# oppo-us-research/PoP-Net

Measured on AMD Instinct MI355X. Metric: depth-frames/sec end-to-end (480x640), higher is better.
Workload: dtype bf16

## Files before the change

### include/popnet_hip.h

```cpp
#ifndef POPNET_HIP_H
#define POPNET_HIP_H

#include <stddef.h>
#include <stdint.h>

#ifdef __cplusplus
extern "C" {
#endif

#define PN_ABI_VERSION 1

enum pn_status {
    PN_OK = 0,
    PN_ERR_INVALID = -1,
    PN_ERR_HIP = -2,
    PN_ERR_STATE = -3,
    PN_ERR_UNSUPPORTED = -4
};

enum pn_precision {
    PN_PREC_F32 = 0,
    PN_PREC_BF16 = 1,
    PN_PREC_BF16X3 = 2
};
// ... 16 lines not shown
int pn_abi_version(void);
int pn_build_experiments(void);
int pn_mfma_sustained(pn_ctx *ctx, double seconds, int waves_per_simd, double *tflops, double *in_kernel_ghz, void *hip_stream);
pn_ctx *pn_create(int device_id);
void pn_destroy(pn_ctx *ctx);
int pn_last_error(pn_ctx *ctx, char *buf, size_t buf_len);

int pn_preprocess(pn_ctx *ctx, const void *depth_dev, int depth_dtype, int B, int H, int W,
                  float *out_dev, int S, float depth_max, float depth_mean, float depth_std,
                  void *hip_stream);

pn_net *pn_net_create(pn_ctx *ctx, int kind, int num_parts, int a, int input_dim);
void pn_net_destroy(pn_net *net);
int pn_net_set_tensor(pn_net *net, const char *name, const float *host_data,
                      const int64_t *shape, int ndim);
int pn_net_finalize(pn_net *net, int precision, int max_batch, int in_h, int in_w);

int pn_rtpose_forward(pn_net *net, const float *x_dev, int B, float *paf_dev, float *heat_dev,
                      float *z_dev, void *hip_stream);
int pn_yolo_forward(pn_net *net, const float *x_dev, int B, float *out_dev, void *hip_stream);
int pn_rtpose_forward_frames(pn_net *net, const void *depth_dev, int depth_dtype, int B, int H, int W, float depth_max,
                             float depth_mean, float depth_std, float *paf_dev, float *heat_dev, float *z_dev,
                             void *hip_stream);
int pn_yolo_forward_frames(pn_net *net, const void *depth_dev, int depth_dtype, int B, int H, int W, float depth_max,
                           float depth_mean, float depth_std, float *out_dev, void *hip_stream);
int pn_net_read_activation(pn_net *net, const char *name, int B, float *host_out,
                           size_t host_elems, void *hip_stream);
int pn_net_copy_activation(pn_net *net, const char *name, int B, float *dev_out, void *hip_stream);
int pn_net_forward_partial(pn_net *net, const float *x_dev, int B, int nsteps, void *hip_stream);
int pn_net_forward_frames_partial(pn_net *net, const void *depth_dev, int depth_dtype, int B, int H, int W, float depth_max,
                                  float depth_mean, float depth_std, int nsteps, void *hip_stream);
int pn_net_num_steps(pn_net *net);
int pn_net_step_info(pn_net *net, int k, char *out, size_t cap);
int pn_conv_level_plan_info(pn_ctx *ctx, int precision, int max_batch, int num_cus, int B, int H, int W, int together, int nconv,
                            const int *cout, const int *cin, const int *ks, const int *stride, char *out, size_t cap);
int pn_conv_has_instance(int prec, int ks, int stride, int pitch, int cfg);
double pn_net_flops_per_frame(pn_net *net);
int pn_net_lock(pn_net *net, int locked);
int pn_net_profile_begin(pn_net *net);
int pn_net_profile_end(pn_net *net, double *conv_ms, int64_t *conv_launches, double *conv_flops,
                       double *other_ms, int64_t *other_launches);
int pn_net_profile_kernel(pn_net *net, int rank, char *name, size_t name_cap, double *ms,
                          int64_t *launches, double *flops);

#define PN_NUM_JOINTS 15
#define PN_NUM_LIMBS 14
#define PN_MAX_PEAKS_PER_JOINT 32
#define PN_MAX_PEAKS (PN_NUM_JOINTS * PN_MAX_PEAKS_PER_JOINT)
#define PN_MAX_CONN_PER_LIMB PN_MAX_PEAKS_PER_JOINT
#define PN_MAX_PERSONS 32

#define PN_FRAME_OVERFLOW_PEAKS 1u
#define PN_FRAME_OVERFLOW_PERSONS 2u

#define PN_Z_READOUT_HEAT_WEIGHTED 0
#define PN_Z_READOUT_CELL 1

typedef struct pn_parse_cfg {
    float thresh_heatmap;
    float thresh_paf;
    int   num_intermed_pts;
    int   downsample;
    int   input_size;
    int   w_org, h_org;
    double fx, fy, cx, cy;
    float depth_mean, depth_std;
// ... 276 lines not shown
```

### popnet_amd/_lib.py

```python
import ctypes as C
import os

import numpy as np

_HERE = os.path.dirname(os.path.abspath(__file__))
LIB_PATH = os.environ.get("POPNET_LIB_PATH") or os.path.join(_HERE, "libpopnet_hip.so")

PN_OK = 0
PN_PREC_F32, PN_PREC_BF16, PN_PREC_BF16X3 = 0, 1, 2
PN_NET_RTPOSE_LIGHT3D, PN_NET_YOLO_POSENET, PN_NET_A2J = 0, 1, 2
PN_DEPTH_F16, PN_DEPTH_F32, PN_DEPTH_NET = 0, 1, 2

PN_NUM_JOINTS = 15
PN_NUM_LIMBS = 14
PN_MAX_PEAKS_PER_JOINT = 32
PN_MAX_PEAKS = PN_NUM_JOINTS * PN_MAX_PEAKS_PER_JOINT
PN_MAX_PERSONS = 32
PN_YOLO_MAX_DET = 64
PN_PLAN_FORWARD, PN_PLAN_DGRAD, PN_PLAN_DGRAD_STRIDED, PN_PLAN_WGRAD = 0, 1, 2, 3
PN_FRAME_OVERFLOW_PEAKS, PN_FRAME_OVERFLOW_PERSONS = 1, 2


class PopnetError(RuntimeError):
    pass
# ... 65 lines not shown

PN_WIRE_MAX_PERSONS = 16
POSE_WIRE_DTYPE = np.dtype([
    ("n_persons", np.int32), ("status", np.uint32),
    ("person_joint", np.int16, (PN_WIRE_MAX_PERSONS, PN_NUM_JOINTS)),
    ("vals", np.float32, (PN_WIRE_MAX_PERSONS, PN_NUM_JOINTS, 6)),
], align=True)

_lib = None

_vp, _i, _f, _d, _sz = C.c_void_p, C.c_int, C.c_float, C.c_double, C.c_size_t
_SIGNATURES = {
    "pn_abi_version": (_i, []),
    "pn_build_experiments": (_i, []),
    "pn_mfma_sustained": (_i, [_vp, _d, _i, C.POINTER(_d), C.POINTER(_d), _vp]),
    "pn_create": (_vp, [_i]),
    "pn_destroy": (None, [_vp]),
    "pn_last_error": (_i, [_vp, C.c_char_p, _sz]),
    "pn_preprocess": (_i, [_vp, _vp, _i, _i, _i, _i, _vp, _i, _f, _f, _f, _vp]),
    "pn_net_create": (_vp, [_vp, _i, _i, _i, _i]),
    "pn_net_destroy": (None, [_vp]),
    "pn_net_set_tensor": (_i, [_vp, C.c_char_p, _vp, C.POINTER(C.c_int64), _i]),
    "pn_net_finalize": (_i, [_vp, _i, _i, _i, _i]),
    "pn_rtpose_forward": (_i, [_vp, _vp, _i, _vp, _vp, _vp, _vp]),
    "pn_yolo_forward": (_i, [_vp, _vp, _i, _vp, _vp]),
    "pn_rtpose_forward_frames": (_i, [_vp, _vp, _i, _i, _i, _i, _f, _f, _f, _vp, _vp, _vp, _vp]),
    "pn_yolo_forward_frames": (_i, [_vp, _vp, _i, _i, _i, _i, _f, _f, _f, _vp, _vp]),
    "pn_net_read_activation": (_i, [_vp, C.c_char_p, _i, _vp, _sz, _vp]),
    "pn_net_copy_activation": (_i, [_vp, C.c_char_p, _i, _vp, _vp]),
    "pn_net_forward_partial": (_i, [_vp, _vp, _i, _i, _vp]),
    "pn_net_forward_frames_partial": (_i, [_vp, _vp, _i, _i, _i, _i, _f, _f, _f, _i, _vp]),
    "pn_net_num_steps": (_i, [_vp]),
    "pn_net_step_info": (_i, [_vp, _i, C.c_char_p, _sz]),
    "pn_conv_level_plan_info": (_i, [_vp] + [_i] * 8 + [_vp] * 4 + [C.c_char_p, _sz]),
    "pn_conv_has_instance": (_i, [_i] * 5),
    "pn_net_flops_per_frame": (_d, [_vp]),
    "pn_net_lock": (_i, [_vp, _i]),
    "pn_parse_reserve": (_i, [_vp, _i]),
    "pn_net_profile_begin": (_i, [_vp]),
    "pn_net_profile_end": (_i, [_vp, C.POINTER(_d), C.POINTER(C.c_int64), C.POINTER(_d), C.POINTER(_d), C.POINTER(C.c_int64)]),
    "pn_net_profile_kernel": (_i, [_vp, _i, C.c_char_p, _sz, C.POINTER(C.c_double), C.POINTER(C.c_int64), C.POINTER(C.c_double)]),
    "pn_parse_cfg_default": (None, [C.POINTER(ParseCfg)]),
    "pn_parse_paf": (_i, [_vp, _vp, _vp, _vp, _i, _i, _i, C.POINTER(ParseCfg), _vp, _vp]),
    "pn_parse_paf_wire": (_i, [_vp, _vp, _vp, _vp, _i, _i, _i, C.POINTER(ParseCfg), _vp, _vp, _vp]),
    "pn_target_cfg_default": (None, [C.POINTER(TargetCfg)]),
    "pn_compose_depth": (_i, [_vp, _vp, _vp, _vp, _vp, _i, _i, _i, _i, _i, _f, _vp, _vp]),
    "pn_compose_bg": (_i, [_vp, _vp, _vp, _vp, _i, _i, _i, _i, _vp, _vp]),
    "pn_rasterize_targets": (_i, [_vp, _vp, _vp, _vp, _i, _i, _vp, C.POINTER(TargetCfg), _vp, _vp, _vp, _vp, _vp]),
    "pn_sizeof_augment_item": (_sz, []),
    "pn_sizeof_parse_cfg": (_sz, []),
    "pn_augment_resize": (_i, [_vp, _vp, _vp, _vp, _i, _i, _i, _vp, _i, _f, _f, _f, _vp]),
    "pn_train_set_precision": (_i, [_vp, _i]),
    "pn_train_ws_keep": (_i, [_vp, _i]),
    "pn_train_pack_cache": (_i, [_vp, _i]),
    "pn_train_pack_refresh": (_i, [_vp, _vp]),
    "pn_conv2d_forward": (_i, [_vp, _vp, _vp, _vp, _vp] + [_i] * 9 + [_vp]),
    "pn_conv2d_dgrad": (_i, [_vp, _vp, _vp, _vp] + [_i] * 8 + [_vp]),
    "pn_conv2d_wgrad": (_i, [_vp, _vp, _vp, _vp, _vp] + [_i] * 8 + [_vp]),
    "pn_bn_train_forward": (_i, [_vp] * 10 + [_f, _f] + [_i] * 4 + [_vp]),
    "pn_bn_train_backward": (_i, [_vp] * 8 + [_i] * 4 + [_vp] * 4 + [_i, _vp]),
    "pn_avgpool3s2_forward": (_i, [_vp, _vp, _vp, _i, _i, _i, _vp]),
    "pn_avgpool3s2_backward": (_i, [_vp, _vp, _vp, _i, _i, _i, _vp]),
    "pn_head_forward": (_i, [_vp, _vp, _vp, _vp] + [_i] * 4 + [_vp, _vp, _i, _vp, _vp]),
    "pn_head_backward": (_i, [_vp, _vp, _vp, _vp, _vp] + [_i] * 5 + [_vp, _vp]),
    "pn_slice_copy": (_i, [_vp, _vp, _i, _vp] + [_i] * 5 + [_vp]),
    "pn_sgd_nesterov": (_i, [_vp, _vp, _vp, _vp, C.c_size_t, _f, _f, _f, _i, _f, _vp]),
# ... 154 lines not shown
```

### popnet_amd/csrc/api.hip

```cpp
#pragma clang fp contract(off)
#include <cmath>
#include <cstdarg>
#include <cstdio>
#include <cstdlib>
#include <cstring>
#include "pn_internal.h"
#include "preproc_pixel.h"

template <typename TIN>
__global__ void preprocess_kernel(const TIN *__restrict__ depth, float *__restrict__ out, int B, int H, int W, int S,
                                  double scale_x, double scale_y, float dmax, float mean, float stdv) {
    const unsigned pix = blockIdx.x * blockDim.x + threadIdx.x;
    if (pix >= (unsigned)(S * S)) return;
    const int b = blockIdx.y;
    const int dy = (int)(pix / (unsigned)S);
    const int dx = (int)(pix - (unsigned)dy * (unsigned)S);
    const size_t gid = (size_t)b * S * S + pix;

    out[gid] = pn_preproc_pixel(depth + (size_t)b * H * W, H, W, dy, dx, scale_x, scale_y, dmax, mean, stdv);
}

PnSwitches pn_read_switches() {
    auto set = [](const char *name) { return getenv(name) != nullptr; };
    auto num = [](const char *name, int unset) { const char *e = getenv(name); return e ? atoi(e) : unset; };
    auto is = [](const char *name, const char *value) { const char *e = getenv(name); return e && !strcmp(e, value); };
    PnSwitches s;
    s.no_conv3 = set("POPNET_NO_CONV3");
    s.conv3_rpg8 = set("POPNET_CONV3_RPG8");
    s.conv3_pt14 = num("POPNET_CONV3_PT14", 0);
    s.conv3_nbuf2 = set("POPNET_CONV3_NBUF2");
    s.generic_c64_off = num("POPNET_GENERIC_C64", 1) == 0;
    if (set("POPNET_CONV4")) s.conv4 = num("POPNET_CONV4", 0) == 0 ? 0 : 1;
    s.no_mix = set("POPNET_NO_MIX");
    s.no_bblock = set("POPNET_NO_BBLOCK");
    s.bblock_x3 = num("POPNET_BBLOCK_X3", 0) != 0;
    s.bb64_static = set("POPNET_BB64_STATIC");
    s.bb64_halves = num("POPNET_BB64_HALVES", 1) == 2 ? 2 : 1;
    if (set("POPNET_BB64_STRIP")) { const int v = num("POPNET_BB64_STRIP", 0); s.bb64_strip = v == 1 || v == 2 ? v : 0; }
    s.no_tailfuse = set("POPNET_NO_TAILFUSE");
    s.no_poolfuse = set("POPNET_NO_POOLFUSE");
    s.no_stempool = set("POPNET_NO_STEMPOOL");
    s.no_embed3 = set("POPNET_NO_EMBED3");
    s.train_x3_wide = set("POPNET_TRAIN_X3_WIDE");
    s.train_wgrad_novec = set("POPNET_TRAIN_WGRAD_NOVEC");
    s.trainx_one_stream = num("POPNET_TRAINX_STREAMS", 0) == 1;
    s.trainx_stem_handover = set("POPNET_TRAINX_STEM_HANDOVER");
    s.trainx_stem_gather = is("POPNET_TRAINX_STEM_FWD", "gather");
    s.trainx_stem_bn_separate = is("POPNET_TRAINX_STEM_BN", "separate");
    s.trainx_stem_depth = num("POPNET_TRAINX_STEM_DEPTH", 2);
    s.trainx_pack_gather = is("POPNET_TRAINX_PACK", "gather");
    s.trainx_legacy_wgrad = is("POPNET_TRAINX_WGRAD", "legacy");
    return s;
}

extern "C" {

int pn_abi_version(void) { return PN_ABI_VERSION; }
int pn_build_experiments(void) { return 0; }

pn_ctx *pn_create(int device_id) {
    pn_ctx *ctx = new pn_ctx();
    ctx->device = device_id;
    int ndev = 0;
    hipError_t e = hipGetDeviceCount(&ndev);
    if (e != hipSuccess || device_id < 0 || device_id >= ndev) {
        char buf[256];
        snprintf(buf, sizeof buf, "pn_create: device %d not available (%d devices, %s)", device_id, ndev,
                 hipGetErrorString(e));
        ctx->err = buf;
        ctx->device = -1;
        return ctx;
    }
    hipDeviceProp_t prop;
    if (hipGetDeviceProperties(&prop, device_id) == hipSuccess) ctx->num_cus = prop.multiProcessorCount;
    return ctx;
// ... 85 lines not shown
```

### popnet_amd/csrc/conv_mfma.hip

```cpp
#include "pn_internal.h"
#include "conv_inst_table.h"

int pn_cfg_couts(int cfg) {
    switch (cfg) {
        case PN_CFG_C128: return 128;
        case PN_CFG_C64: return 64;
        case PN_CFG_C64W: return 64;
        case PN_CFG_C32: return 32;
        default: return 16;
    }
}


int pn_cfg_pixels(int cfg) { return cfg == PN_CFG_C128 ? 112 : (cfg == PN_CFG_C64W ? 224 : 128); }

size_t pn_conv_lds_bytes(int prec, int ks, int stride, int pitch, int R, int dil) {
    size_t pixb = prec == PN_PREC_BF16 ? 128 : 256;
    size_t rows = (size_t)(R - 1) * stride + (size_t)(ks - 1) * dil + 1;
    return rows * pitch * pixb;
}

extern "C" int pn_conv_has_instance(int prec, int ks, int stride, int pitch, int cfg) {
    if (prec != PN_PREC_BF16 && prec != PN_PREC_F32) return 0;
#define PN_HAS_CASE(KS, ST, PITCH, CFG) \
    if (ks == KS && stride == ST && pitch == PITCH && cfg == CFG) return 1;
    PN_CONV_INSTANCES(PN_HAS_CASE)
#undef PN_HAS_CASE
    return 0;
}

int pn_conv_has_instance_d2(int prec, int ks, int stride, int pitch, int cfg) {
    if (prec != PN_PREC_BF16 && prec != PN_PREC_F32) return 0;
#define PN_HAS_CASE(KS, ST, PITCH, CFG) \
    if (ks == KS && stride == ST && pitch == PITCH && cfg == CFG) return 1;
    PN_CONV_INSTANCES_D2(PN_HAS_CASE)
#undef PN_HAS_CASE
    return 0;
}

int pn_launch_conv_part0(pn_ctx *ctx, const ConvLaunch &L, hipStream_t stream);
int pn_launch_conv_d2_part0(pn_ctx *ctx, const ConvLaunch &L, hipStream_t stream);
int pn_launch_conv_d2_part1(pn_ctx *ctx, const ConvLaunch &L, hipStream_t stream);
int pn_launch_conv_acc_part0(pn_ctx *ctx, const ConvLaunch &L, hipStream_t stream);
int pn_launch_conv_acc_part1(pn_ctx *ctx, const ConvLaunch &L, hipStream_t stream);
int pn_launch_conv_acc_part2(pn_ctx *ctx, const ConvLaunch &L, hipStream_t stream);
int pn_launch_conv_part1(pn_ctx *ctx, const ConvLaunch &L, hipStream_t stream);
int pn_launch_conv_part2(pn_ctx *ctx, const ConvLaunch &L, hipStream_t stream);
int pn_launch_conv_part3(pn_ctx *ctx, const ConvLaunch &L, hipStream_t stream);

int pn_launch_conv(pn_ctx *ctx, const ConvLaunch &L, hipStream_t stream) {
    int rc;
    if (L.kern == 4) return pn_launch_conv4(ctx, L, stream);
    if (L.kern == 3) return pn_launch_conv3(ctx, L, stream);
    if (L.acc) {
        if (L.prec == PN_PREC_F32 && (L.dil == 1 || L.dil == 2)) {
            if ((rc = pn_launch_conv_acc_part0(ctx, L, stream)) != 1) return rc;
            if ((rc = pn_launch_conv_acc_part1(ctx, L, stream)) != 1) return rc;
            if ((rc = pn_launch_conv_acc_part2(ctx, L, stream)) != 1) return rc;
        }
        return pn_set_error(ctx, PN_ERR_UNSUPPORTED, "no blocked-accumulation conv kernel for prec=%d ks=%d stride=%d dilation=%d pitch=%d cfg=%d", L.prec, L.ks, L.stride, L.dil, L.pitch, L.cfg);
    }
    if (L.dil != 1) {
        if (L.dil == 2 && (rc = pn_launch_conv_d2_part0(ctx, L, stream)) != 1) return rc;
        if (L.dil == 2 && (rc = pn_launch_conv_d2_part1(ctx, L, stream)) != 1) return rc;
        return pn_set_error(ctx, PN_ERR_UNSUPPORTED, "no conv kernel for prec=%d ks=%d stride=%d dilation=%d pitch=%d cfg=%d", L.prec, L.ks, L.stride, L.dil, L.pitch, L.cfg);
    }
    if ((rc = pn_launch_conv_part0(ctx, L, stream)) != 1) return rc;
    if ((rc = pn_launch_conv_part1(ctx, L, stream)) != 1) return rc;
    if ((rc = pn_launch_conv_part2(ctx, L, stream)) != 1) return rc;
    if ((rc = pn_launch_conv_part3(ctx, L, stream)) != 1) return rc;
    return pn_set_error(ctx, PN_ERR_UNSUPPORTED, "no conv kernel for prec=%d ks=%d stride=%d pitch=%d cfg=%d", L.prec, L.ks,
                        L.stride, L.pitch, L.cfg);
}

int pn_conv_stage_maxpx(int prec, int ks, int stride, int pitch, int cfg) {
    if (cfg == PN_CFG_C64W) return 0;
    const int maxpx = stride != 1 ? 0 : (ks == 1 ? 128 : (pitch <= 32 ? 192 : (pitch <= 64 ? 288 : 360)));
    const int nch = prec == PN_PREC_BF16 ? 8 : 16;
    const int raw = (maxpx * nch + 255) / 256;
    return raw <= 12 ? maxpx : 0;
}
```

### popnet_amd/csrc/net_api.hip

```cpp
#include <cstdarg>
#include <cstdio>
#include <cstring>
#include "net_internal.h"

using namespace pnnet;

namespace {
std::string geom_json(int prec, bool x3, const ConvGeom &g, int H, int W, int cout, int cin_chunks, int B) {
    ConvProblem P;
    memset(&P, 0, sizeof P);
    pn_fill_conv_problem(P, {nullptr, H, W, 0, 64, 0}, B, cin_chunks, cout, g, prec, x3);
    char t[384];
    snprintf(t, sizeof t, "\"kernel\": \"%s\", \"kern\": %d, \"cfg\": %d, \"pitch\": %d, \"R\": %d, \"Wt\": %d, \"wc\": %d, \"wp\": %d, \"nbuf\": %d, \"pt\": %d, \"rpg\": %d, "
             "\"tiles_x\": %d, \"tiles_per_img\": %d, \"cout_blocks\": %d, \"nblocks\": %d, \"lds_two\": %d",
             (g.dil != 1 ? pn_conv_kernel_label_dil(prec, g.ks, g.stride, g.pitch, g.cfg, g.dil) : pn_conv_kernel_label(prec, g.kern, false, g.ks, g.stride, g.pitch, g.cfg, g.wc, g.wp, g.nbuf, g.pt, g.rpg)).c_str(), g.kern, g.cfg, g.pitch, g.R, g.Wt, g.wc,
             g.wp, g.nbuf, g.pt, g.rpg, P.tiles_x, P.tiles_per_img, P.cout_blocks, P.nblocks, P.lds_two);
    return t;
}

int forward_entry(pn_net *n, int kind, bool pointers_ok, bool state = true) {
    if (!n) return PN_ERR_INVALID;
    pn_ctx *ctx = n->ctx;
    if (n->kind != kind)
        return pn_set_error(ctx, PN_ERR_INVALID, "not %s net", kind == PN_NET_RTPOSE_LIGHT3D ? "an rtpose_light3d" : kind == PN_NET_YOLO_POSENET ? "a YoloPoseNet" : "an A2J");
// ... 238 lines not shown
        else js += "null";
        const Buf &ib = n->bufs[c.in_buf];
        js += ", " + geom_json(n->prec, n->x3, c, ib.H, ib.W, c.cout, c.cin_chunks, n->last_B > 0 ? n->last_B : n->max_batch);
        if (c.dil != 1) add(", \"dil\": %d", c.dil);
        if (c.acc) add(", \"blocked_acc\": %d", c.acc);
        js += "}";
    };
    if (k == -1) {
        add("{\"prec\": \"%s\", \"in_h\": %d, \"in_w\": %d, \"input_dim\": %d, \"max_batch\": %d, \"steps\": %zu, \"bufs\": [",
            n->x3 ? "bf16x3" : n->prec == PN_PREC_BF16 ? "bf16" : "fp32", n->in_h, n->in_w, n->input_dim, n->max_batch, n->steps.size());
        for (size_t i = 0; i < n->bufs.size(); ++i) add(i ? ", [%d, %d, %d]" : "[%d, %d, %d]", n->bufs[i].H, n->bufs[i].W, n->bufs[i].plane);
        js += "]}";
    } else {
        const Step &st = n->steps[k];
        static const char *types[] = {"stem", "pool", "conv", "bblock"};
        add("{\"type\": \"%s\", \"kernel\": \"%s\"", types[(int)st.type], step_label(n, st).c_str());
        if (st.type == Step::STEM) add(", \"cin\": %d, \"out_buf\": %d, \"pool_buf\": %d", st.stem_cin, st.out_buf, st.stem_pool_buf);
        else if (st.type == Step::POOL) add(", \"mode\": %d, \"in_buf\": %d, \"out_buf\": %d, \"C\": %d, \"out_coff\": %d", st.pool.mode, st.pool.in_buf, st.pool.out_buf, st.pool.C, st.pool.out_coff);
        else {
            js += ", \"convs\": [";
            for (size_t i = 0; i < st.conv_ids.size(); ++i) {
                if (i) js += ", ";
                conv(st.conv_ids[i]);
            }
            js += "]";
        }
        js += "}";
    }
    if (js.size() + 1 > cap) return pn_set_error(ctx, PN_ERR_INVALID, "pn_net_step_info: %zu bytes needed", js.size() + 1);
    memcpy(out, js.c_str(), js.size() + 1);
    return PN_OK;
}

int pn_conv_level_plan_info(pn_ctx *ctx, int precision, int max_batch, int num_cus, int B, int H, int W, int together, int nconv, const int *cout,
                            const int *cin, const int *ks, const int *stride, char *out, size_t cap) {
    if (!ctx) return PN_ERR_INVALID;
    if (!out || !cout || !cin || !ks || !stride || nconv < 1 || nconv > 3 || max_batch < 1 || B < 1 || B > max_batch || num_cus < 1 || H < 1 || W < 1 ||
        (precision != PN_PREC_F32 && precision != PN_PREC_BF16 && precision != PN_PREC_BF16X3))
        return pn_set_error(ctx, PN_ERR_INVALID, "pn_conv_level_plan_info: bad arguments");
    for (int i = 0; i < nconv; ++i)
        if (cout[i] < 1 || cin[i] < 1 || (ks[i] != 1 && ks[i] != 3) || (stride[i] != 1 && stride[i] != 2))
            return pn_set_error(ctx, PN_ERR_INVALID, "pn_conv_level_plan_info: convolution %d: bad arguments", i);
    const bool x3 = precision == PN_PREC_BF16X3;
    const int prec = x3 ? PN_PREC_BF16 : precision;
    const PnSwitches sw = pn_read_switches();
    std::vector<PnLevelConv> lv(nconv);
    for (int i = 0; i < nconv; ++i) {
        lv[i].H = H; lv[i].W = W; lv[i].rows = cout[i]; lv[i].ks = ks[i]; lv[i].stride = stride[i];
        lv[i].cin_gt64 = cin[i] > 64;
    }
    if (together) pn_plan_level(lv, max_batch, x3, sw.conv4);
    std::string js = "{\"convs\": [";
    for (int i = 0; i < nconv; ++i) {
        const int cin_chunks = ((x3 ? 3 : 1) * cin[i] + 63) / 64;
        ConvGeom g;
        g.ks = ks[i]; g.stride = stride[i];
        pn_plan_conv_kernel(prec, max_batch, num_cus, H, W, cout[i], cin_chunks, lv[i].wc_min, lv[i].nbuf_min, lv[i].k4_level, sw, g);
        const char *why = "";
        if (int rc = pn_plan_conv_tiles(prec, H, W, g, &why)) return pn_set_error(ctx, rc, "conv %d: %s", i, why);
        js += (i ? ", {" : "{") + geom_json(prec, x3, g, H, W, cout[i], cin_chunks, B) + "}";
    }
    js += "]}";
    if (js.size() + 1 > cap) return pn_set_error(ctx, PN_ERR_INVALID, "pn_conv_level_plan_info: %zu bytes needed", js.size() + 1);
    memcpy(out, js.c_str(), js.size() + 1);
    return PN_OK;
}
// ... 12 lines not shown
```

### popnet_amd/csrc/net_internal.h

```cpp
#pragma once
#include <map>
#include <string>
#include <vector>
#include "pn_internal.h"
#include "conv_plan.h"
#include "preproc_pixel.h"

namespace pnnet {
struct HostTensor {
    std::vector<int64_t> shape;
    std::vector<float> data;
    size_t numel() const { return data.size(); }
};

struct Buf {
    void *p = nullptr;
    int H = 0, W = 0, C = 0;
    int plane = 0;
    size_t bytes = 0;
};

struct Image {
    std::vector<unsigned char> host;
    size_t bytes = 0;
// ... 72 lines not shown
    double flops_per_frame = 0;
    int out_h = 0, out_w = 0;
    bool profiling = false;
    std::map<std::string, pnnet::ProfRow> prof_by_kernel;
    std::vector<pnnet::ProfRec> prof;
    size_t prof_used = 0;
    PnFrameSrc frame_src = {};

    size_t esize() const { return prec == PN_PREC_BF16 ? 2 : 4; }
    void *dev(int image) const { return image < 0 ? nullptr : images[image].dev; }
};

namespace pnnet {
inline const HostTensor *find_t(const pn_net *n, const std::string &name) {
    auto it = n->tensors.find(name);
    return it == n->tensors.end() ? nullptr : &it->second;
}
inline int add_image(pn_net *n, const void *data, size_t bytes) {
    n->images.emplace_back();
    n->images.back().bytes = bytes;
    if (data) n->images.back().host.assign((const unsigned char *)data, (const unsigned char *)data + bytes);
    return (int)n->images.size() - 1;
}
template <class T> int add_image(pn_net *n, const std::vector<T> &v) { return add_image(n, v.data(), v.size() * sizeof(T)); }

int compile_net(pn_net *n);
int prepare_conv(pn_net *n, ConvSpec &cs);
int pack_stem(pn_net *n, Step &st, const std::string &conv, const std::string &bn, int sum_cin);
int pack_bblock(pn_net *n, Step &st);
int pack_tail(pn_net *n, ConvSpec &a);
int upload_net(pn_net *n);
void release_net(pn_net *n);
bool level_is_mixed(const pn_net *n, const Step &st);
std::string step_label(const pn_net *n, const Step &st);
int run_forward(pn_net *n, const float *x, int B, hipStream_t stream, int nsteps = -1);
}
```

### popnet_amd/csrc/net_run.hip

```cpp
#include <algorithm>
#include <cstring>
#include "net_internal.h"

namespace pnnet {
int upload_net(pn_net *n) {
    pn_ctx *ctx = n->ctx;
    PN_HIP_CHECK(ctx, hipSetDevice(ctx->device));
    for (auto &b : n->bufs) {
        PN_HIP_CHECK(ctx, hipMalloc(&b.p, b.bytes + 2048));
        PN_HIP_CHECK(ctx, hipMemset(b.p, 0, b.bytes + 2048));
    }
    for (auto &im : n->images) {
        PN_HIP_CHECK(ctx, hipMalloc(&im.dev, im.bytes));
        if (im.host.empty()) PN_HIP_CHECK(ctx, hipMemset(im.dev, 0, im.bytes));
        else PN_HIP_CHECK(ctx, hipMemcpy(im.dev, im.host.data(), im.bytes, hipMemcpyHostToDevice));
    }
    PN_HIP_CHECK(ctx, hipDeviceSynchronize());
    return PN_OK;
}

void release_net(pn_net *n) {
    for (auto &b : n->bufs) if (b.p) (void)hipFree(b.p);
    for (auto &im : n->images) if (im.dev) (void)hipFree(im.dev);
    for (auto &r : n->prof) { (void)hipEventDestroy(r.a); (void)hipEventDestroy(r.b); }
}

bool level_is_mixed(const pn_net *n, const Step &st) {
    const ConvSpec &c0 = n->convs[st.conv_ids[0]];
    for (int id : st.conv_ids)
        if (c0.kern == 3 && (n->convs[id].ks != c0.ks || (n->convs[id].tail_conv >= 0) != (c0.tail_conv >= 0))) return true;
    return false;
}

std::string step_label(const pn_net *n, const Step &st) {
    if (st.type == Step::STEM) {
        if (st.stem_pool_buf >= 0) return "stem7x7_pool_kernel";
        if (st.stem_cin > 1) return "conv2d_forward+nchw_relu_to_nhwc_kernel";
        if (n->prec == PN_PREC_F32) return "stem7x7_kernel";
        return n->x3 ? "stem7x7_mfma_kernel<x3>" : "stem7x7_mfma_kernel";
    }
    if (st.type == Step::POOL) return pn_pool_kernel_label(st.pool.mode, n->x3);
    if (st.type == Step::BBLOCK) return n->x3 ? "bb64x3_kernel" : "bb64_kernel";
    const ConvSpec &c0 = n->convs[st.conv_ids[0]];
    if (c0.dil != 1) return pn_conv_kernel_label_dil(n->prec, c0.ks, c0.stride, c0.pitch, c0.cfg, c0.dil);
    return pn_conv_kernel_label(n->prec, c0.kern, level_is_mixed(n, st), c0.ks, c0.stride, c0.pitch, c0.cfg, c0.wc, c0.wp, c0.nbuf, c0.pt, c0.rpg);
}

namespace {
int refresh_problems(pn_net *n, int B, hipStream_t stream) {
    for (auto &st : n->steps) {
        if (st.type != Step::CONV) continue;
        const ConvSpec &c0 = n->convs[st.conv_ids[0]];
        st.host_probs.clear();
        int max_blocks = 0;
        bool two_bufs = false, has_tail = false, pool_tail = false;
        for (int id : st.conv_ids) {
            const ConvSpec &cs = n->convs[id];
            const Buf &ib = n->bufs[cs.in_buf];
            if (n->x3 && ib.plane % 64)
                return pn_set_error(n->ctx, PN_ERR_UNSUPPORTED, "bf16x3: input plane of %d channels is not a multiple of 64 (the K loop wraps to the hi plane per 64-channel chunk)", ib.plane);
            ConvProblem P;
            memset(&P, 0, sizeof P);
            pn_fill_conv_problem(P, {ib.p, ib.H, ib.W, ib.C, ib.plane, ib.bytes}, B, cs.cin_chunks, cs.cout, cs, n->prec, n->x3);
            P.wpack = n->dev(cs.wpack);
            P.bias = (const float *)n->dev(cs.bias);
            P.in_coff = cs.in_coff;
            if (cs.out_buf >= 0) { P.out = n->bufs[cs.out_buf].p; P.out_cs = n->bufs[cs.out_buf].C; P.out_coff = cs.out_coff; P.split = n->x3 ? n->bufs[cs.out_buf].plane : 0; }
            if (cs.res_buf >= 0) { P.res = n->bufs[cs.res_buf].p; P.res_cs = n->bufs[cs.res_buf].C; P.res_coff = cs.res_coff; P.res_split = n->x3 ? n->bufs[cs.res_buf].plane : 0; }
            if (cs.nchw_slot >= 0) P.out_nchw = n->nchw_ptr[cs.nchw_slot];
            P.act = cs.act;
            P.yolo_naf = 5 + 3 * n->num_parts;
            if (cs.pool_tail) {
                const Buf &pb = n->bufs[cs.pool_out_buf];
                P.tiles_x = (pb.W + 6) / 7;
                P.tiles_per_img = ((pb.H + 2) / 3) * P.tiles_x;
                P.nblocks = B * P.tiles_per_img * P.cout_blocks;
                P.tail_out = pb.p; P.tail_out_cs = pb.C; P.tail_out_coff = cs.pool_out_coff;
                P.tail_split = n->x3 ? pb.plane : 0;
                P.out = nullptr;
                pool_tail = true;
            }
            if (cs.tail_conv >= 0) {
                const ConvSpec &tb = n->convs[cs.tail_conv];
                P.tail_w = n->dev(cs.tail_wpack); P.tail_bias = (const float *)n->dev(cs.tail_bias); P.tail_cout = tb.cout; P.tail_act = tb.act;
                if (tb.out_buf >= 0) { P.tail_out = n->bufs[tb.out_buf].p; P.tail_out_cs = n->bufs[tb.out_buf].C; P.tail_out_coff = tb.out_coff; }
                if (tb.nchw_slot >= 0) P.tail_nchw = n->nchw_ptr[tb.nchw_slot];
                P.out = nullptr;
                has_tail = true;
            }
            if (P.lds_two) two_bufs = true;
            max_blocks = std::max(max_blocks, P.nblocks);
            st.host_probs.push_back(P);
        }
        pn_fill_conv_launch(st.launch, n->prec, c0, (int)st.host_probs.size(), max_blocks, two_bufs);
        if (c0.kern == 3) {
            st.launch.tail = has_tail ? 1 : pool_tail ? 2 : 0;
            if (level_is_mixed(n, st)) st.launch.mix = 1;
            for (int id : st.conv_ids) {
                const ConvSpec &cs = n->convs[id];
                st.launch.lds_bytes = std::max(st.launch.lds_bytes, pn_conv3_lds_bytes(cs.ks, cs.wp, cs.nbuf, cs.rpg));
            }
            if (st.launch.tail == 1) st.launch.lds_bytes = std::max<size_t>(st.launch.lds_bytes, 4 * 7 * 1024 + 1024);
            if (st.launch.tail == 2 && n->x3) st.launch.lds_bytes = std::max<size_t>(st.launch.lds_bytes, 2 * 4 * 7 * 1024);
        }
        st.launch.probs_dev = (const ConvProblem *)n->dev(st.dev_probs);
        PN_HIP_CHECK(n->ctx, hipMemcpyAsync(n->dev(st.dev_probs), st.host_probs.data(), st.host_probs.size() * sizeof(ConvProblem),
                                            hipMemcpyHostToDevice, stream));
    }
    n->last_B = B;
    for (int i = 0; i < 4; ++i) n->last_nchw[i] = n->nchw_ptr[i];
    return PN_OK;
}

int profile_step(pn_net *n, const Step &st, int B, hipStream_t stream, ProfRec **out) {
    pn_ctx *ctx = n->ctx;
    if (n->prof_used == n->prof.size()) {
        ProfRec r;
        PN_HIP_CHECK(ctx, hipEventCreate(&r.a));
        PN_HIP_CHECK(ctx, hipEventCreate(&r.b));
        n->prof.push_back(r);
    }
    ProfRec *pr = &n->prof[n->prof_used++];
    const bool conv = st.type == Step::CONV || st.type == Step::BBLOCK;
    pr->kind = conv ? (int)Step::CONV : (int)st.type;
    pr->flops = 0;
    for (int id : st.conv_ids) pr->flops += n->convs[id].flops * B;
    pr->label = conv ? step_label(n, st) : std::string();
    PN_HIP_CHECK(ctx, hipEventRecord(pr->a, stream));
    *out = pr;
    return PN_OK;
}
}

int run_forward(pn_net *n, const float *x, int B, hipStream_t stream, int nsteps) {
    pn_ctx *ctx = n->ctx;
    if (B < 1 || B > n->max_batch) return pn_set_error(ctx, PN_ERR_INVALID, "batch %d outside [1, %d]", B, n->max_batch);
    bool dirty = B != n->last_B;
// ... 119 lines not shown
```

### popnet_amd/csrc/pn_internal.h

```cpp
#pragma once
#include <hip/hip_runtime.h>
#include <stdint.h>
#include <string.h>
#include <string>
#include <vector>
#include "../../include/popnet_hip.h"

enum PnPackKind { PN_PACK_TILE3 = 0, PN_PACK_TILE3_X3 = 1, PN_PACK_C1_X3 = 2 };

struct pn_ctx {
    int device = 0;
    std::string err;
    int num_cus = 256;
    void *parse_ws = nullptr;
    size_t parse_ws_bytes = 0;
    bool parse_ws_fixed = false;
    int parse_last_b = 0;
    void *parse_big = nullptr;
    void *train_ws = nullptr;
    size_t train_ws_bytes = 0;
    bool train_ws_keep = false;
    std::vector<void *> train_ws_retired;
    bool train_lds_attr = false;
    bool train_x3 = false;
    struct PackEntry { const float *w; int Cout, Cin, flip; PnPackKind kind; void *buf; size_t bytes; bool fresh; };
    bool train_pack_cache = false;
    std::vector<PackEntry> train_packs;
    void *train_pack_table = nullptr;
    size_t train_pack_table_entries = 0;
    size_t train_pack_table_cap = 0;
    unsigned train_pack_blocks = 0;
};

struct PnSwitches {
    bool no_conv3 = false;
    bool conv3_rpg8 = false;
    int conv3_pt14 = 0;
    bool conv3_nbuf2 = false;
    bool generic_c64_off = false;
    int conv4 = -1;
    bool no_mix = false;
    bool no_bblock = false;
    bool bblock_x3 = false;
    bool bb64_static = false;
    int bb64_halves = 1;
    int bb64_strip = -1;
    bool no_tailfuse = false;
    bool no_poolfuse = false;
    bool no_stempool = false;
    bool no_embed3 = false;
    bool train_x3_wide = false;
    bool train_wgrad_novec = false;
    bool trainx_one_stream = false;
    bool trainx_stem_handover = false;
    bool trainx_stem_gather = false;
    bool trainx_stem_bn_separate = false;
    int trainx_stem_depth = 2;
    bool trainx_pack_gather = false;
    bool trainx_legacy_wgrad = false;
};
PnSwitches pn_read_switches();

int pn_set_error(pn_ctx *ctx, int code, const char *fmt, ...);

inline uint16_t pn_f32_to_bf16(float f) {
    uint32_t u;
    memcpy(&u, &f, 4);
    if ((u & 0x7fffffffu) > 0x7f800000u) return (uint16_t)((u >> 16) | 0x40);
    u += 0x7fffu + ((u >> 16) & 1u);
    return (uint16_t)(u >> 16);
}
inline float pn_bf16_to_f32(uint16_t h) { const uint32_t u = (uint32_t)h << 16; float f; memcpy(&f, &u, 4); return f; }
void pn_parse_big_free(pn_ctx *ctx);

__host__ __device__ inline int pn_limb_src(int l) {
    constexpr int t[PN_NUM_LIMBS] = {8, 9, 11, 8, 10, 12, 8, 1, 2, 4, 1, 3, 5, 1};
    return t[l];
}
__host__ __device__ inline int pn_limb_dst(int l) {
    constexpr int t[PN_NUM_LIMBS] = {9, 11, 13, 10, 12, 14, 1, 2, 4, 6, 3, 5, 7, 0};
    return t[l];
}
int pn_train_ws(pn_ctx *ctx, size_t bytes, void **out);
// ... 64 lines not shown
    const void *tail_w;
    const float *tail_bias;
    void *tail_out;
    float *tail_nchw;
    int tail_cout, tail_act, tail_out_cs, tail_out_coff;
    int tail_split;
};

enum pn_conv_cfg {
    PN_CFG_C128 = 0,
    PN_CFG_C64 = 1,
    PN_CFG_C32 = 2,
    PN_CFG_C16 = 3,
    PN_CFG_C64W = 4
};
int pn_cfg_couts(int cfg);
inline int pn_cfg_ct(int cfg) { return cfg == PN_CFG_C16 ? 1 : 2; }
inline int pn_conv_row_channel(int tile, int row, int CT) {
    return (tile / CT) * CT * 16 + 4 * CT * (row >> 2) + 4 * (tile % CT) + (row & 3);
}
int pn_cfg_pixels(int cfg);

struct ConvLaunch {
    int prec;
    int ks;
    int stride;
    int pitch;
    int cfg;
    int kern = 0, wc = 0, wp = 0, nbuf = 0, pt = 7, rpg = 4;
    int dil = 1;
    int acc = 0;
    int tail = 0;
    int mix = 0;
    int nprob;
    int max_blocks;
    size_t lds_bytes;
    const ConvProblem *probs_dev;
};
int pn_launch_conv(pn_ctx *ctx, const ConvLaunch &L, hipStream_t stream);
inline std::string pn_conv_kernel_label(int prec, int kern, bool mix, int ks, int stride, int pitch, int cfg, int wc, int wp, int nbuf, int pt, int rpg) {
    char lb[96];
    if (kern == 4) snprintf(lb, sizeof lb, "conv4_kernel");
    else if (kern == 3 && mix) snprintf(lb, sizeof lb, "conv3_mix_kernel");
    else if (kern == 3) snprintf(lb, sizeof lb, "conv3_kernel<%d, %d, %d, %d, %d, %d>", ks, wc, wp, nbuf, pt, rpg);
    else snprintf(lb, sizeof lb, "conv_mfma_kernel<%d, %d, %d, %d, %d>", prec, ks, stride, pitch, cfg);
    return lb;
}
inline std::string pn_conv_kernel_label_dil(int prec, int ks, int stride, int pitch, int cfg, int dil) {
    char lb[96];
    snprintf(lb, sizeof lb, "conv_mfma_kernel<%d, %d, %d, %d, %d, %d>", prec, ks, stride, pitch, cfg, dil);
    return lb;
}
inline std::string pn_pool_kernel_label(int mode, bool split) {
    char lb[48];
    snprintf(lb, sizeof lb, "pool_kernel<%d%s>", mode, split ? ", split" : "");
    return lb;
}
int pn_launch_conv3(pn_ctx *ctx, const ConvLaunch &L, hipStream_t stream);
int pn_launch_conv4(pn_ctx *ctx, const ConvLaunch &L, hipStream_t stream);

struct BBProblem {
    const void *in;
    void *out;
    const void *wpack;
    const float *bias1, *bias2;
    int B, H, W;
    int in_cs, in_coff, out_cs, out_coff;
    int Wt, tiles_x, tiles_per_img, ntiles;
    unsigned in_zero_off;
    int in_split, out_split;
    int *tickets;
    int halves;
    int strip_S, strip_T, nseg;
};
int pn_launch_bb64(pn_ctx *ctx, const BBProblem &P, hipStream_t stream);
int pn_launch_bb64s(pn_ctx *ctx, const BBProblem &P, hipStream_t stream);
int pn_launch_bb64x3(pn_ctx *ctx, const BBProblem &P, hipStream_t stream);
size_t pn_conv3_lds_bytes(int ks, int WP, int nbuf, int rpg = 4);
size_t pn_conv_lds_bytes(int prec, int ks, int stride, int pitch, int R, int dil = 1);
int pn_conv_has_instance_d2(int prec, int ks, int stride, int pitch, int cfg);
constexpr size_t PN_CONV_LDS_MAX = 160 * 1024;
int pn_conv_stage_maxpx(int prec, int ks, int stride, int pitch, int cfg);

struct PnFrameSrc;
int pn_launch_stem_pool(pn_ctx *ctx, const float *x, const void *wfrag, const float *bias, void *out, int B, int H, int W, int Ho, int Wo,
                        int out_cs, hipStream_t stream, const PnFrameSrc *src);
struct PnFrameSrc;
int pn_launch_stem(pn_ctx *ctx, int prec, const float *x, const float *w, const void *wfrag, const float *bias,
                   void *out, int B, int H, int W, int Ho, int Wo, int out_cs, int split, hipStream_t stream, const PnFrameSrc *src = nullptr);

int pn_launch_pool(pn_ctx *ctx, int prec, int mode, const void *in, void *out, int B, int H, int W,
                   int C, int in_cs, int out_cs, int out_coff, int in_split, int out_split, hipStream_t stream);
// ... 14 lines not shown
```

Baseline: 69850.

## Add specialized head conv kernel for small 3x3 bf16 levels

Adds a dedicated MFMA kernel for 3x3 stride-1 bf16 convolution levels with at most 32 output channels and one or two input chunks, typical of the network heads. It loads the whole halo tile for all input chunks into LDS once, keeps a register queue of weight fragments, and schedules MFMAs with explicit group barriers. Tiles are re-planned to 4 rows by up to 30 columns, giving many small blocks in place of the generic kernel's tiling. This adds a separate code path that can be disabled by an environment switch and may lose occupancy on large LDS footprints.

```diff
diff --git a/include/popnet_hip.h b/include/popnet_hip.h
--- a/include/popnet_hip.h
+++ b/include/popnet_hip.h
@@ -72,6 +72,7 @@
                                   float depth_mean, float depth_std, int nsteps, void *hip_stream);
 int pn_net_num_steps(pn_net *net);
 int pn_net_step_info(pn_net *net, int k, char *out, size_t cap);
+int pn_net_step_head_kernel(pn_net *net, int k);
 int pn_conv_level_plan_info(pn_ctx *ctx, int precision, int max_batch, int num_cus, int B, int H, int W, int together, int nconv,
                             const int *cout, const int *cin, const int *ks, const int *stride, char *out, size_t cap);
 int pn_conv_has_instance(int prec, int ks, int stride, int pitch, int cfg);
diff --git a/popnet_amd/_lib.py b/popnet_amd/_lib.py
--- a/popnet_amd/_lib.py
+++ b/popnet_amd/_lib.py
@@ -121,6 +121,7 @@
     "pn_net_forward_frames_partial": (_i, [_vp, _vp, _i, _i, _i, _i, _f, _f, _f, _i, _vp]),
     "pn_net_num_steps": (_i, [_vp]),
     "pn_net_step_info": (_i, [_vp, _i, C.c_char_p, _sz]),
+    "pn_net_step_head_kernel": (_i, [_vp, _i]),
     "pn_conv_level_plan_info": (_i, [_vp] + [_i] * 8 + [_vp] * 4 + [C.c_char_p, _sz]),
     "pn_conv_has_instance": (_i, [_i] * 5),
     "pn_net_flops_per_frame": (_d, [_vp]),
diff --git a/popnet_amd/csrc/api.hip b/popnet_amd/csrc/api.hip
--- a/popnet_amd/csrc/api.hip
+++ b/popnet_amd/csrc/api.hip
@@ -41,6 +41,7 @@
     s.no_poolfuse = set("POPNET_NO_POOLFUSE");
     s.no_stempool = set("POPNET_NO_STEMPOOL");
     s.no_embed3 = set("POPNET_NO_EMBED3");
+    s.no_headk = set("POPNET_NO_HEADK");
     s.train_x3_wide = set("POPNET_TRAIN_X3_WIDE");
     s.train_wgrad_novec = set("POPNET_TRAIN_WGRAD_NOVEC");
     s.trainx_one_stream = num("POPNET_TRAINX_STREAMS", 0) == 1;
diff --git a/popnet_amd/csrc/conv_mfma.hip b/popnet_amd/csrc/conv_mfma.hip
--- a/popnet_amd/csrc/conv_mfma.hip
+++ b/popnet_amd/csrc/conv_mfma.hip
@@ -50,6 +50,7 @@
 
 int pn_launch_conv(pn_ctx *ctx, const ConvLaunch &L, hipStream_t stream) {
     int rc;
+    if (L.headk) return pn_launch_headk(ctx, L, stream);
     if (L.kern == 4) return pn_launch_conv4(ctx, L, stream);
     if (L.kern == 3) return pn_launch_conv3(ctx, L, stream);
     if (L.acc) {
diff --git a/popnet_amd/csrc/headk_inst.hip b/popnet_amd/csrc/headk_inst.hip
--- /dev/null
+++ b/popnet_amd/csrc/headk_inst.hip
@@ -0,0 +1,3 @@
+#include "headk_kernel.h"
+
+int pn_launch_headk(pn_ctx *ctx, const ConvLaunch &L, hipStream_t stream) { return headk_launch(ctx, L, stream); }
diff --git a/popnet_amd/csrc/headk_kernel.h b/popnet_amd/csrc/headk_kernel.h
--- /dev/null
+++ b/popnet_amd/csrc/headk_kernel.h
@@ -0,0 +1,132 @@
+#pragma once
+#include "conv_common.h"
+
+#define PNH_QUART (6 * 32 * 32)
+#define PNH_HALF (2 * PNH_QUART)
+
+template <int CT>
+__global__ __launch_bounds__(256, 3) void headk_kernel(const ConvProblem *__restrict__ probs) {
+    typedef __bf16 T;
+    constexpr int KS = 3, KK = 9, PT = 2, FRAGB = 1024;
+    extern __shared__ __attribute__((aligned(16))) char smem[];
+
+    const ConvProblem &P = probs[blockIdx.y];
+    if ((int)blockIdx.x >= P.nblocks) return;
+    const int bx = pn_xcd_block(blockIdx.x, P.nblocks);
+    const int tid = threadIdx.x;
+    const int lane = tid & 63;
+    const int wave = __builtin_amdgcn_readfirstlane(tid >> 6);
+    const int c = lane & 15, q = lane >> 4;
+
+    const int Wo = P.Wo;
+    const PnTile tl = pn_tile_decode(bx, P.tiles_per_img, P.tiles_x, P.R, P.Wt, P.Ho, Wo);
+    const int b = tl.b, oy0 = tl.oy0, ox0 = tl.ox0, Wc = tl.Wc, npix = tl.npix;
+    const int HC = Wc + KS - 1;
+    const int iy0 = oy0 - 1, ix0 = ox0 - 1;
+    const float inv_wc = tl.inv_wc;
+    const int nchunks = P.cin_chunks;
+
+    const size_t frame_b = ((size_t)b * P.H * P.W * P.in_cs + P.in_coff) * 2;
+    const char *img = (const char *)P.in + frame_b;
+    const unsigned zero_rel = P.in_zero_off - (unsigned)frame_b;
+    const int qd = wave & 1, row0 = (wave >> 1) * 3;
+    unsigned boff[3];
+#pragma unroll
+    for (int j = 0; j < 3; ++j) {
+        const int px = lane >> 1;
+        const int iy = iy0 + row0 + j, ix = ix0 + px;
+        const bool inb = px < HC && (unsigned)ix < (unsigned)P.W && (unsigned)iy < (unsigned)P.H;
+        boff[j] = inb ? (unsigned)((iy * P.W + ix) * P.in_cs * 2 + qd * 32 + (lane & 1) * 16) : zero_rel;
+    }
+    const unsigned dst0 = (unsigned)__builtin_amdgcn_readfirstlane(qd * PNH_QUART + row0 * 1024);
+    for (int hh = 0; hh < 2 * nchunks; ++hh) {
+#pragma unroll
+        for (int j = 0; j < 3; ++j) pn_glds16_s<0>(img + (size_t)hh * 64, boff[j], dst0 + (unsigned)(hh * PNH_HALF + j * 1024));
+    }
+
+    constexpr int NSTEP = KK * 2;
+    constexpr int NA = 9, DB = 6;
+    constexpr int NITEM = NSTEP * PT;
+    static_assert(NSTEP % NA == 0 && NITEM % DB == 0, "queue slot of an item must not depend on the chunk");
+    const __amdgpu_buffer_rsrc_t wrsrc = pn_weight_rsrc(P.wpack);
+    unsigned wbase[CT], wlast[CT];
+    pn_weight_bases<CT>(0, P.ksteps, FRAGB, wbase);
+#pragma unroll
+    for (int ct = 0; ct < CT; ++ct) wlast[ct] = wbase[ct] + (unsigned)__builtin_amdgcn_readfirstlane((P.ksteps - 1) * FRAGB);
+    const unsigned wlane = (unsigned)lane * 16u;
+    auto load_w = [&](int ct) {
+        const bf16x8 f = __builtin_bit_cast(bf16x8, __builtin_amdgcn_raw_buffer_load_b128(wrsrc, wlane, min(wbase[ct], wlast[ct]), 0));
+        wbase[ct] += FRAGB;
+        return f;
+    };
+    bf16x8 aq[NA][CT];
+#pragma unroll
+    for (int d = 0; d < NA - 1; ++d)
+#pragma unroll
+        for (int ct = 0; ct < CT; ++ct) aq[d][ct] = load_w(ct);
+
+    int baddr[PT];
+#pragma unroll
+    for (int pt = 0; pt < PT; ++pt) {
+        const int slot = (wave * PT + pt) * 16 + c;
+        const int s = slot < npix ? slot : 0;
+        int ry, rx;
+        pn_slot_pixel(s, inv_wc, Wc, ry, rx);
+        baddr[pt] = (q >> 1) * PNH_QUART + (q & 1) * 16 + (ry * 32 + rx) * 32;
+    }
+    f32x4 acc[CT][PT];
+#pragma unroll
+    for (int ct = 0; ct < CT; ++ct)
+#pragma unroll
+        for (int pt = 0; pt < PT; ++pt) acc[ct][pt] = f32x4{0.f, 0.f, 0.f, 0.f};
+
+    asm volatile("s_waitcnt vmcnt(0)\n\ts_barrier" ::: "memory");
+
+#define PNH_BOFF(j) ((((j) / PT) / KK) * PNH_HALF + (((((j) / PT) % KK) / KS) * 32 + (((j) / PT) % KK) % KS) * 32)
+    for (int chunk = 0; chunk < nchunks; ++chunk) {
+        bf16x8 bq[DB];
+#pragma unroll
+        for (int j = 0; j < DB - 1; ++j) bq[j] = *reinterpret_cast<const bf16x8 *>(smem + baddr[j % PT] + PNH_BOFF(j));
+        __builtin_amdgcn_sched_barrier(0);
+#pragma clang loop unroll(full)
+        for (int j = 0; j < NITEM; ++j) {
+            const int s = j / PT, pt = j % PT, jr = j + DB - 1;
+            if (pt == 0) {
+#pragma unroll
+                for (int ct = 0; ct < CT; ++ct) aq[(s + NA - 1) % NA][ct] = load_w(ct);
+            }
+            if (jr < NITEM) bq[jr % DB] = *reinterpret_cast<const bf16x8 *>(smem + baddr[jr % PT] + PNH_BOFF(jr));
+#pragma unroll
+            for (int ct = 0; ct < CT; ++ct) acc[ct][pt] = __builtin_amdgcn_mfma_f32_16x16x32_bf16(aq[s % NA][ct], bq[j % DB], acc[ct][pt], 0, 0, 0);
+            if (pt == 0) __builtin_amdgcn_sched_group_barrier(0x020, CT, 0);
+            if (jr < NITEM) __builtin_amdgcn_sched_group_barrier(0x100, 1, 0);
+            __builtin_amdgcn_sched_group_barrier(0x008, CT, 0);
+        }
+        __builtin_amdgcn_sched_barrier(0);
+#pragma unroll
+        for (int pt = 0; pt < PT; ++pt) baddr[pt] += 2 * PNH_HALF;
+    }
+#undef PNH_BOFF
+
+    constexpr int LC = CT * 4;
+    const int cw = LC * q;
+    const int cout = P.cout, act = P.act;
+    float bias[LC];
+    pn_load_bias<LC>(P.bias, cw, bias);
+    PN_GLOBAL T *out_base = P.out ? (PN_GLOBAL T *)P.out + P.out_coff + cw : nullptr;
+    PN_GLOBAL float *nchw = (PN_GLOBAL float *)P.out_nchw;
+    const int out_cs = P.out_cs, Ho = P.Ho, naf = P.yolo_naf;
+    const int pix0 = (b * Ho + oy0) * Wo + ox0;
+    pn_with_act<true>(act, [&](auto actc) {
+        pn_conv_epilogue<decltype(actc)::value, T, CT, PT>(acc, bias, wave * PT * 16 + c, npix, inv_wc, Wc, cw, cout, act, naf, (const PN_GLOBAL T *)nullptr, 0, 0,
+                                                           out_base, out_cs, 0, nchw, b, Ho, Wo, oy0, ox0, pix0);
+    });
+}
+
+static int headk_launch(pn_ctx *ctx, const ConvLaunch &L, hipStream_t stream) {
+    if (L.lds_bytes > 4 * PNH_HALF) return pn_set_error(ctx, PN_ERR_UNSUPPORTED, "head kernel: halo image of %zu B", L.lds_bytes);
+    if (L.cfg == PN_CFG_C16) hipLaunchKernelGGL(headk_kernel<1>, dim3(L.max_blocks, L.nprob), dim3(256), L.lds_bytes, stream, L.probs_dev);
+    else hipLaunchKernelGGL(headk_kernel<2>, dim3(L.max_blocks, L.nprob), dim3(256), L.lds_bytes, stream, L.probs_dev);
+    PN_HIP_CHECK(ctx, hipGetLastError());
+    return PN_OK;
+}
diff --git a/popnet_amd/csrc/net_api.hip b/popnet_amd/csrc/net_api.hip
--- a/popnet_amd/csrc/net_api.hip
+++ b/popnet_amd/csrc/net_api.hip
@@ -294,6 +294,13 @@
     return PN_OK;
 }
 
+int pn_net_step_head_kernel(pn_net *n, int k) {
+    if (!n) return PN_ERR_INVALID;
+    if (!n->finalized) return pn_set_error(n->ctx, PN_ERR_STATE, "net not finalized");
+    if (k < 0 || k >= (int)n->steps.size()) return pn_set_error(n->ctx, PN_ERR_INVALID, "step %d outside [0, %zu)", k, n->steps.size());
+    return head_level(n, n->steps[k]) ? 1 : 0;
+}
+
 int pn_conv_level_plan_info(pn_ctx *ctx, int precision, int max_batch, int num_cus, int B, int H, int W, int together, int nconv, const int *cout,
                             const int *cin, const int *ks, const int *stride, char *out, size_t cap) {
     if (!ctx) return PN_ERR_INVALID;
diff --git a/popnet_amd/csrc/net_internal.h b/popnet_amd/csrc/net_internal.h
--- a/popnet_amd/csrc/net_internal.h
+++ b/popnet_amd/csrc/net_internal.h
@@ -128,6 +128,7 @@
 int upload_net(pn_net *n);
 void release_net(pn_net *n);
 bool level_is_mixed(const pn_net *n, const Step &st);
+bool head_level(const pn_net *n, const Step &st);
 std::string step_label(const pn_net *n, const Step &st);
 int run_forward(pn_net *n, const float *x, int B, hipStream_t stream, int nsteps = -1);
 }
diff --git a/popnet_amd/csrc/net_run.hip b/popnet_amd/csrc/net_run.hip
--- a/popnet_amd/csrc/net_run.hip
+++ b/popnet_amd/csrc/net_run.hip
@@ -44,6 +44,19 @@
     const ConvSpec &c0 = n->convs[st.conv_ids[0]];
     if (c0.dil != 1) return pn_conv_kernel_label_dil(n->prec, c0.ks, c0.stride, c0.pitch, c0.cfg, c0.dil);
     return pn_conv_kernel_label(n->prec, c0.kern, level_is_mixed(n, st), c0.ks, c0.stride, c0.pitch, c0.cfg, c0.wc, c0.wp, c0.nbuf, c0.pt, c0.rpg);
+}
+
+bool head_level(const pn_net *n, const Step &st) {
+    if (n->sw.no_headk || n->prec != PN_PREC_BF16 || n->x3 || st.type != Step::CONV) return false;
+    const int cfg = n->convs[st.conv_ids[0]].cfg;
+    if (cfg != PN_CFG_C16 && cfg != PN_CFG_C32) return false;
+    for (int id : st.conv_ids) {
+        const ConvSpec &cs = n->convs[id];
+        if (cs.ks != 3 || cs.stride != 1 || cs.dil != 1 || cs.acc || cs.kern != 0 || cs.cfg != cfg) return false;
+        if (cs.cout > 32 || cs.res_buf >= 0 || cs.tail_conv >= 0 || cs.pool_tail) return false;
+        if (cs.cin_chunks != 1 && cs.cin_chunks != 2) return false;
+    }
+    return true;
 }
 
 namespace {
@@ -103,6 +116,21 @@
             if (st.launch.tail == 1) st.launch.lds_bytes = std::max<size_t>(st.launch.lds_bytes, 4 * 7 * 1024 + 1024);
             if (st.launch.tail == 2 && n->x3) st.launch.lds_bytes = std::max<size_t>(st.launch.lds_bytes, 2 * 4 * 7 * 1024);
         }
+        st.launch.headk = head_level(n, st) ? 1 : 0;
+        if (st.launch.headk) {
+            st.launch.max_blocks = 0;
+            st.launch.lds_bytes = 0;
+            for (ConvProblem &P : st.host_probs) {
+                const int segs = (P.Wo + 29) / 30;
+                P.Wt = (P.Wo + segs - 1) / segs;
+                P.R = std::min(P.Ho, 4);
+                P.tiles_x = (P.Wo + P.Wt - 1) / P.Wt;
+                P.tiles_per_img = ((P.Ho + P.R - 1) / P.R) * P.tiles_x;
+                P.nblocks = B * P.tiles_per_img;
+                st.launch.max_blocks = std::max(st.launch.max_blocks, P.nblocks);
+                st.launch.lds_bytes = std::max<size_t>(st.launch.lds_bytes, (size_t)P.cin_chunks * 2 * 12288);
+            }
+        }
         st.launch.probs_dev = (const ConvProblem *)n->dev(st.dev_probs);
         PN_HIP_CHECK(n->ctx, hipMemcpyAsync(n->dev(st.dev_probs), st.host_probs.data(), st.host_probs.size() * sizeof(ConvProblem),
                                             hipMemcpyHostToDevice, stream));
diff --git a/popnet_amd/csrc/pn_internal.h b/popnet_amd/csrc/pn_internal.h
--- a/popnet_amd/csrc/pn_internal.h
+++ b/popnet_amd/csrc/pn_internal.h
@@ -49,6 +49,7 @@
     bool no_poolfuse = false;
     bool no_stempool = false;
     bool no_embed3 = false;
+    bool no_headk = false;
     bool train_x3_wide = false;
     bool train_wgrad_novec = false;
     bool trainx_one_stream = false;
@@ -179,6 +180,7 @@
     int acc = 0;
     int tail = 0;
     int mix = 0;
+    int headk = 0;
     int nprob;
     int max_blocks;
     size_t lds_bytes;
@@ -205,6 +207,7 @@
 }
 int pn_launch_conv3(pn_ctx *ctx, const ConvLaunch &L, hipStream_t stream);
 int pn_launch_conv4(pn_ctx *ctx, const ConvLaunch &L, hipStream_t stream);
+int pn_launch_headk(pn_ctx *ctx, const ConvLaunch &L, hipStream_t stream);
 
 struct BBProblem {
     const void *in;
```

Result: no change. 69890, median of 2 (+0.1%).
